# HKUST-KnowComp/DualMessagePassing

Measured on AMD Instinct MI355X. Metric: (pattern,graph) pairs/sec DMPNN fwd+bwd hid=128, higher is better.
Workload: dtype f32

## Files before the change

dualmessagepassing_amd/_abi.py:

```python
import ctypes

c_int = ctypes.c_int
c_i32 = ctypes.c_int32
c_i64 = ctypes.c_int64
c_u64 = ctypes.c_uint64
c_f32 = ctypes.c_float
c_double = ctypes.c_double
c_ptr = ctypes.c_void_p
c_size = ctypes.c_size_t

ABI_VERSION = 92

DMP_COLLATE_MAX_JOBS = 4
DMP_POOL_MAX_JOBS = 4
DMP_REDUCE_MAX_SEGMENTS = 16
DMP_ADAMW_MAX_SKIP = 16
DMP_ADAMW_MAX_SEGMENTS = 1024
DMP_LOOKUP_MAX_JOBS = 8
DMP_CONCAT_MAX_JOBS = 12
DMP_GEMM_MAX_JOBS = 12
DMP_GEMM_MAX_TERMS = 3
DMP_ATB_MAX_JOBS = 8
DMP_MEM_MEAN, DMP_MEM_SUM, DMP_MEM_MAX = 0, 1, 2


class dmp_collate_job(ctypes.Structure):
    _fields_ = [("local_src", c_ptr), ("local_dst", c_ptr), ("num_nodes", c_ptr), ("num_edges", c_ptr), ("B", c_i64), ("N", c_i64),
                ("E", c_i64), ("node_off", c_ptr), ("edge_off", c_ptr), ("src", c_ptr), ("dst", c_ptr), ("edge_graph", c_ptr),
                ("node_graph", c_ptr)]


class dmp_pool_job(ctypes.Structure):
    _fields_ = [("sizes_a", c_ptr), ("sizes_b", c_ptr), ("Ba", c_i64), ("Bb", c_i64), ("flag_a", c_ptr), ("flag_b", c_ptr),
                ("rows_a", c_i64), ("R", c_i64), ("chunk", c_int), ("off", c_ptr), ("gptr", c_ptr), ("vptr", c_ptr), ("vent", c_ptr),
                ("gent", c_ptr), ("seg", c_ptr), ("flag8", c_ptr), ("rowmap", c_ptr), ("sizes", c_ptr)]


class dmp_smallk_job(ctypes.Structure):
    _fields_ = [("X", c_ptr), ("ldx", c_i64), ("D", c_ptr), ("ldd", c_i64), ("gate", c_ptr), ("rowmask", c_ptr), ("R", c_i64),
                ("partial", c_ptr)]


class dmp_l0_pack_job(ctypes.Structure):
    _fields_ = [("enc_p", c_ptr), ("ldp", c_i64), ("rows_p", c_i64), ("enc_g", c_ptr), ("ldg", c_i64), ("gate", c_ptr), ("rows_g", c_i64),
# ... 244 lines not shown
    "dmp_mfma_partial_rows_h": (c_i64, [c_i64, c_int]),
    "dmp_gemm_k64": (c_int, [c_ptr, c_i64, c_ptr, c_i64, c_int, c_ptr, c_i64, c_i64, c_ptr]),
    "dmp_atb_typed": (c_int, [c_ptr, c_i64, c_ptr, c_i64, c_ptr, c_ptr, c_ptr, c_i64, c_i64, c_int, c_ptr, c_ptr, c_ptr]),
    "dmp_out_fwd_fused_rows": (c_int, [c_ptr, c_i64, c_ptr, c_i64, c_ptr, c_ptr, c_ptr, c_int, c_ptr, c_i64, c_i64, c_int, c_int, c_ptr,
                                       c_i64, c_ptr]),
    "dmp_bwd_h1_fused_rows": (c_int, [c_ptr, c_i64, c_ptr, c_i64, c_ptr, c_i64, c_ptr, c_ptr, c_ptr, c_int, c_i64, c_int, c_f32, c_ptr,
                                      c_i64, c_ptr, c_ptr, c_ptr]),
    "dmp_kept_rows_scratch_words": (c_i64, [c_i64]),
    "dmp_kept_rows": (c_int, [c_ptr, c_i64, c_int, c_ptr, c_ptr, c_ptr, c_ptr]),
    "dmp_l0_edge_fwd_rows": (c_int, [c_ptr, c_i64, c_int, c_ptr, c_i64, c_ptr, c_i64, c_ptr, c_ptr, c_ptr, c_ptr, c_ptr, c_ptr, c_i64, c_int,
                                     c_f32, c_ptr, c_i64, c_ptr]),
    "dmp_l0_bwd_w_rows": (c_int, [c_ptr, c_i64, c_int, c_ptr, c_ptr, c_i64, c_ptr, c_i64, c_ptr, c_ptr, c_i64, c_int, c_ptr, c_ptr]),
    "dmp_typed_partial_rows": (c_i64, [c_i64, c_int]),
    "dmp_out_fwd_typed": (c_int, [_p(dmp_typed_job), c_int, c_ptr, c_ptr, c_ptr, c_i64, c_i64, c_int, c_ptr]),
    "dmp_bwd_h1_typed": (c_int, [c_ptr, c_i64, c_ptr, c_i64, c_ptr, c_i64, c_ptr, c_ptr, c_ptr, c_i64, c_i64, c_int, c_f32, c_ptr, c_i64,
                                 c_ptr, c_ptr, c_ptr]),
    "dmp_kept_rows_jobs": (c_int, [_p(dmp_kept_job), c_int, c_ptr, c_ptr, c_ptr, c_ptr, c_i64, c_ptr, c_ptr, c_ptr, c_ptr]),
    "dmp_row_mask_bits_jobs": (c_int, [_p(dmp_rowmask_job), c_int, c_ptr]),
    "dmp_atb2_blocks": (c_i64, [c_i64, c_int]),
    "dmp_atb2_jobs": (c_int, [_p(dmp_atb2_job), c_int, c_ptr, c_ptr, c_ptr, c_i64, c_i64, c_int, c_ptr]),
    "dmp_bwd_z_w": (c_int, [c_ptr, c_i64, c_ptr, c_i64, c_ptr, c_i64, c_ptr, c_i64, c_i64, c_ptr, c_i64, c_ptr, c_ptr, c_f32, c_f32,
                            c_ptr, c_ptr, c_ptr, c_i64, c_i64, c_int, c_ptr, c_i64, c_ptr, c_i64, c_ptr, c_ptr]),
    "dmp_out_fwd_typed_codes": (c_int, [_p(dmp_typed_job), c_ptr, c_i64, c_int, c_ptr, c_i64, c_i64, c_i64, c_ptr, c_ptr, c_ptr, c_i64, c_i64, c_int, c_ptr]),
    "dmp_bwd_h1_w_blocks": (c_i64, [c_i64]),
    "dmp_bwd_h1_w": (c_int, [c_ptr, c_i64, c_ptr, c_i64, c_ptr, c_i64, c_ptr, c_ptr, c_i64, c_i64, c_int, c_f32, c_ptr, c_i64,
                             c_ptr, c_ptr, c_ptr, c_ptr]),
    "dmp_node_chain_blocks": (c_i64, [c_i64]),
    "dmp_node_chain_panel_words": (c_i64, []),
    "dmp_node_chain_pack": (c_int, [_p(dmp_chain_panel), c_int, c_ptr, c_ptr]),
    "dmp_node_chain_fwd": (c_int, [c_ptr, c_i64, c_ptr, c_i64, c_ptr, c_ptr, c_ptr, c_int, c_f32, c_ptr, c_ptr, c_i64, c_i64, c_int,
                                   c_ptr, c_i64, c_ptr, c_i64, c_ptr, c_i64, c_ptr]),
    "dmp_node_chain_bwd": (c_int, [c_ptr, c_i64, c_ptr, c_i64, c_ptr, c_i64, c_ptr, c_int, c_f32, c_ptr, c_ptr, c_i64, c_i64, c_int,
                                   c_ptr, c_i64, c_ptr, c_i64, c_ptr, c_i64, c_ptr, c_ptr, c_ptr]),
    "dmp_row_mask_bits": (c_int, [c_ptr, c_i64, c_ptr, c_ptr]),
    "dmp_row_mask_rows": (c_int, [c_ptr, c_i64, c_int, c_i64, c_ptr, c_ptr]),
    "dmp_bwd_z_fused": (c_int, [c_ptr, c_i64, c_ptr, c_i64, c_ptr, c_i64, c_i64, c_ptr, c_i64, c_ptr, c_ptr, c_ptr,
                                c_f32, c_f32, c_i64, c_int, c_ptr, c_i64, c_ptr]),
    "dmp_gemm_k128": (c_int, [c_ptr, c_i64, c_ptr, c_i64, c_int, c_ptr, c_i64, c_i64, c_int, c_ptr]),
    "dmp_edge_combine": (c_int, [c_ptr, c_i64, c_ptr, c_i64, c_ptr, c_ptr, c_ptr, c_ptr, c_ptr, c_i64,
                                 c_int, c_int, c_f32, c_ptr, c_i64, c_ptr]),
    "dmp_relu_bwd_g_colsum": (c_int, [c_ptr, c_i64, c_ptr, c_i64, c_ptr, c_ptr, c_i64, c_int, c_f32, c_ptr, c_i64,
                                      c_ptr, c_ptr]),
    "dmp_edge_combine_bwd_g": (c_int, [c_ptr, c_i64, c_ptr, c_ptr, c_i64, c_int, c_ptr, c_i64, c_ptr]),
    "dmp_compgcn_agg": (c_int, [c_ptr, c_i64, c_ptr, c_i64, c_ptr, c_ptr, c_ptr, c_ptr, c_i64, c_int, c_int,
                                c_ptr, c_i64, c_ptr]),
    "dmp_compgcn_agg_bwd": (c_int, [c_ptr, c_i64, c_ptr, c_i64, c_ptr, c_i64, c_ptr, c_ptr, c_ptr, c_ptr,
                                    c_i64, c_int, c_int, c_ptr, c_i64, c_ptr, c_i64, c_ptr]),
    "dmp_attn_supported_dh": (c_int, [c_int]),
    "dmp_attn_fwd": (c_int, [c_ptr, c_ptr, c_ptr, c_ptr, c_ptr, c_i64, c_i64, c_i64, c_int, c_int, c_f32, c_ptr, c_ptr, c_ptr, c_ptr]),
    "dmp_attn_bwd": (c_int, [c_ptr, c_ptr, c_ptr, c_ptr, c_ptr, c_ptr, c_ptr, c_ptr, c_i64, c_i64, c_i64, c_int, c_int, c_f32, c_ptr,
                             c_ptr, c_ptr, c_ptr, c_ptr]),
    "dmp_mem_init_fwd": (c_int, [c_ptr, c_i64, c_ptr, c_i64, c_ptr, c_i64, c_i64, c_int, c_int, c_int, c_int, c_int, c_ptr, c_ptr,
                                 c_ptr, c_ptr, c_ptr, c_ptr, c_ptr]),
    "dmp_mem_init_bwd": (c_int, [c_ptr, c_ptr, c_ptr, c_ptr, c_ptr, c_i64, c_i64, c_int, c_int, c_int, c_int, c_ptr, c_ptr, c_ptr]),
    "dmp_cnn_fwd": (c_int, [c_ptr, c_i64, c_i64, c_int, c_ptr, c_ptr, c_int, c_int, c_int, c_int, c_int, c_f32, c_ptr, c_int, c_ptr,
                            c_ptr, c_ptr, c_ptr, c_ptr]),
    "dmp_cnn_route_bwd": (c_int, [c_ptr, c_ptr, c_ptr, c_i64, c_i64, c_i64, c_int, c_int, c_int, c_f32, c_ptr, c_ptr]),
    "dmp_cnn_wgrad_chunks": (c_i64, [c_i64]),
    "dmp_cnn_wgrad": (c_int, [c_ptr, c_ptr, c_i64, c_i64, c_i64, c_int, c_int, c_int, c_ptr, c_ptr]),
    "dmp_rnn_fwd": (c_int, [c_ptr, c_ptr, c_ptr, c_ptr, c_ptr, c_i64, c_i64, c_int, c_int, c_int, c_ptr, c_ptr, c_ptr, c_ptr]),
    "dmp_rnn_bwd": (c_int, [c_ptr, c_ptr, c_ptr, c_ptr, c_ptr, c_i64, c_i64, c_int, c_int, c_int, c_ptr, c_ptr]),
    "dmp_relconv_supported": (c_int, [c_int, c_int]),
    "dmp_relconv_fwd": (c_int, [c_ptr, c_ptr, c_ptr, c_ptr, c_ptr, c_ptr, c_ptr, c_i64, c_int, c_int, c_int, c_int, c_int, c_ptr,
                                c_ptr]),
    "dmp_relconv_bwd": (c_int, [c_ptr, c_ptr, c_ptr, c_ptr, c_ptr, c_ptr, c_ptr, c_i64, c_int, c_int, c_int, c_int, c_int, c_ptr,
                                c_ptr]),
# ... 6 lines not shown
```

dualmessagepassing_amd/_build.py:

```python
import fcntl
import hashlib
import os
import shutil
import subprocess
import tempfile

_HERE = os.path.dirname(os.path.abspath(__file__))
CSRC = os.path.join(_HERE, "csrc")
LIB_PATH = os.path.join(CSRC, "libdmp_hip.so")
HASH_PATH = LIB_PATH + ".srchash"
SOURCES = ["dmp_agg.hip", "dmp_segacc.hip", "dmp_compact.hip", "dmp_graph.hip", "dmp_fused.hip", "dmp_mfma.hip", "dmp_typed.hip", "dmp_h1w.hip", "dmp_nodechain.hip", "dmp_atb.hip", "dmp_fold.hip", "dmp_heads.hip", "dmp_layer0.hip", "dmp_bn.hip", "dmp_attn.hip", "dmp_mem.hip", "dmp_cnn.hip", "dmp_rnn.hip", "dmp_relconv.hip", "dmp_relcorr.hip",
           "dmp_subiso.cpp"]
HEADERS = ["dmp_common.h", "dmp_mfma_common.h", os.path.join("..", "..", "include", "dmp_hip.h")]
ARCH = "gfx950"
FLAGS = ["-O3", "-std=c++17", "-fPIC", "-ffp-contract=off", "-Wall", "-Wno-unused-function"]


def find_hipcc():
    for cand in (os.environ.get("HIPCC"), shutil.which("hipcc"), "/opt/rocm/bin/hipcc"):
        if cand and os.path.exists(cand):
            return cand
    return None


def source_hash():
    h = hashlib.sha256()
    h.update((ARCH + " ".join(FLAGS)).encode())
    for f in SOURCES + HEADERS:
        with open(os.path.join(CSRC, f), "rb") as fh:
            h.update(f.encode())
            h.update(fh.read())
    return h.hexdigest()


def _stale():
    if not os.path.exists(LIB_PATH) or not os.path.exists(HASH_PATH):
        return True
    with open(HASH_PATH) as f:
        return f.read().strip() != source_hash()


def build_lib(force=False, verbose=False):
    if not force and not _stale():
        return LIB_PATH
# ... 43 lines not shown
```

dualmessagepassing_amd/fused.py:

```python
import threading

import torch
from torch.autograd.function import once_differentiable

from . import _abi, _lib, ops
from ._lib import check, ptr, stream_ptr


def _partials(rows, H, dev):
    lib = _lib.load()
    return torch.empty((int(lib.dmp_colsum_partial_rows(rows, H)), H), dtype=torch.float32, device=dev)


MAX_REDUCE_SEGMENTS = _abi.DMP_REDUCE_MAX_SEGMENTS


class _Deferred(threading.local):

    def __init__(self):
        self.stack = []


_deferred = _Deferred()

# ... 617 lines not shown
USE_OUT_CODES = True


def out_codes_ok(h1, enc, K, Wc):
    lib = _lib.load()
    lim = (1 << 32) - 65536
    return bool(USE_OUT_CODES and h1.size(1) == 128 and not lib.dmp_dev_get_exact_fp32() and 1 <= K <= 16 and Wc.size(0) == K and Wc.size(1) == 128
                and enc.dtype == torch.float32 and enc.stride(1) == 1 and enc.stride(0) % 4 == 0 and enc.data_ptr() % 16 == 0
                and enc.size(0) == h1.size(0) and h1.size(0) * 128 * 4 < lim and Wc.stride(1) == 1)


def out_fwd_typed_codes(h1, W2t, b2, enc, K, Wc, tiles, prev=None, out=None, w_in_out=True, row0=0):
    lib = _lib.load()
    slot_edge, tile_scale, num_tiles, bound = tiles
    R, H = h1.shape
    if out is None:
        out = dead_rows_buffer((R, H), h1.device)
    Wc = Wc.detach()
    _lib.require_gpu(h1, W2t, out, prev, b2, enc, Wc)
    j = _abi.dmp_typed_job()
    j.Hin, j.ldh, j.W2, j.ldw, j.w_in_out = h1.data_ptr(), h1.stride(0), W2t.data_ptr(), W2t.stride(0), int(bool(w_in_out))
    j.bias = ptr(b2)
    j.R, j.ldr = ptr(prev), (prev.stride(0) if prev is not None else H)
    j.R2, j.ldr2 = None, H
    j.act, j.slope = 0, 0.0
    j.out, j.ldo = out.data_ptr(), out.stride(0)
    with _lib.timed("out_fwd_typed_codes[H=%d,R=%d]", (H, R), 4 * H * R * 2 + 4 * enc.size(1) * R):
        check(lib.dmp_out_fwd_typed_codes(_ctypes.byref(j), ptr(enc), enc.stride(0), int(K), ptr(Wc), Wc.stride(0), int(row0),
                                          0 if prev is None else min(R, prev.size(0)), ptr(slot_edge), ptr(tile_scale),
                                          ptr(num_tiles), bound, R, H, stream_ptr()), "dmp_out_fwd_typed_codes")
    return out


def out_fwd_typed(h1, W2t, b2, prev, tiles, out=None, w_in_out=True, slope=None, prev2=None):
    R, H = h1.shape
    if out is None:
        out = dead_rows_buffer((R, H), h1.device)
    typed_jobs([dict(a=h1, W=W2t, bias=b2, prev=prev, prev2=prev2, out=out, w_in_out=w_in_out, slope=slope)], tiles)
    return out


def bwd_h1_typed(d_o, W2, h1, tiles, slope=0.0, out=None):
    lib = _lib.load()
    E, H = d_o.shape
    slot_edge, tile_scale, num_tiles, bound = tiles
    d_g = out if out is not None else dead_rows_buffer((E, H), d_o.device)
    G = int(lib.dmp_typed_partial_rows(bound, H))
    part = torch.empty((G, H), dtype=torch.float32, device=d_o.device)
    part_rows = torch.empty_like(part)
    W2 = W2.contiguous()
    with _lib.timed("bwd_h1_typed[H=%d,E=%d]", (H, E), 12 * H * E + 4 * E):
        check(lib.dmp_bwd_h1_typed(ptr(d_o), d_o.stride(0), ptr(W2), W2.size(1), ptr(h1), h1.stride(0), ptr(slot_edge), ptr(tile_scale),
                                   ptr(num_tiles), bound, E, H, slope, ptr(d_g), d_g.stride(0), ptr(part), ptr(part_rows), stream_ptr()),
              "dmp_bwd_h1_typed")
    return d_g, reduce_partials(part), reduce_partials(part_rows)


USE_NODE_CHAIN = True


def node_chain_ok(H, *tensors):
    if not USE_NODE_CHAIN or H != 128 or _lib.load().dmp_dev_get_exact_fp32():
        return False
    lim = (1 << 32) - 65536
    for a in tensors:
        if a is None:
            continue
        if (a.dtype != torch.float32 or a.dim() != 2 or a.stride(1) != 1 or a.stride(0) % 4 or a.stride(0) * 4 > 16383
                or a.data_ptr() % 16 or a.size(0) * a.stride(0) * 4 >= lim):
            return False
    return True

# ... 853 lines not shown
                out_fwd_typed(S[:, H:], Bn[H:], None, XP[:, :H], T, out=H1n, slope=slope, prev2=T1)
        elif l0 is not None and node_pass:
            pass
        elif l0 is not None and l0.venc is not None:
            VK = l0.VK
            XP = torch.empty((N, 3 * H), dtype=torch.float32, device=z.device)
            for t, (n0, n1) in l0.vtables(N):
                smallk_embed(l0.venc[n0:n1, :VK], MV[t * VK:(t + 1) * VK], None, XP[n0:n1], H)
        else:
            XP = x @ Wx
        if (l0 is not None and node_pass) or chained:
            PXr, ldpx = PX, 2 * H
        else:
            PXr, ldpx = XP[:, H:], 3 * H
            if l0 is not None or nd is None:
                H1n = add_bias_relu_(SB, XP[:, :H], bn, slope)
        if chained:
            pass
        elif nd is not None:
            xn = dead_rows_buffer((N, H), z.device) if (inner & 1) else torch.zeros((N, H), dtype=torch.float32, device=z.device)
            if nW2t is not None:
                out_fwd_typed(H1n, nW2t, nb2, x if residual else None, nd.tiles, out=xn)
            else:
                out_fwd_typed(H1n, nW2, nb2, x if residual else None, nd.tiles, out=xn, w_in_out=False)
        elif onepanel_ok(H):
            xn = out_fwd_mfma(H1n, nW2, nb2, v_gate, x if residual else None, nW2t)
        else:
            xn = gate_residual(x if residual else None, torch.addmm(nb2, H1n, nW2.t()), v_gate)
        sums_only = epool is not None and not edge_rows
        zn = None
        side.wait("erows" if l0 is not None else "tiles")
        dead_gate = e_gate if (SKIP_DEAD_ROWS and USE_ROW_MASKS and e_gate is not None and typed_ok(index, H)
                               and gate_row_mask(e_gate) is not None) else None
        if l0 is not None:
            H1e = dead_rows_buffer((z.size(0), H), z.device) if dead_gate is not None else torch.empty((z.size(0), H), dtype=torch.float32, device=z.device)
            for t, rows, _ in tables:
                if rows[1] > rows[0]:
                    l0_edge_fwd(enc0, K0, M0[t * K0:(t + 1) * K0], PXr, ldpx, be, coef, index, slope, rows, H1e,
                                mask=gate_row_mask(dead_gate) if dead_gate is not None else None)
        elif typed_ok(index, H):
            H1e = edge_fwd_typed(z, Wes, PXr, ldpx, be, coef, index, slope, dead_gate=dead_gate, sel=None if nd is None else nd.sel)
        elif mfma_ok(index, H):
            H1e = edge_fwd_mfma(z, Wes, PXr, ldpx, be, coef, index, slope)
        else:
            G = z @ Wes
            H1e = edge_combine_raw(G, 2 * H, PXr, ldpx, be, coef, index, H, relu=True, slope=slope)
            del G
            if not sums_only:
                Oe = torch.addmm(eb2, H1e, eW2.t())
                zn = gate_residual(z if residual else None, Oe, e_gate)
        if zn is None and not sums_only:
            dead = (3 if (inner & 1) else 1) if (dead_gate is not None and zero_rows_gate(e_gate)) else 0
            side.wait("tiles")
            lt = live_tiles(index, coef, e_gate) if (dead == 3 and eW2t is not None) else None
            if lt is not None:
                tl_ = ascending_tiles(e_gate) or lt
                if l0 is not None and residual and getattr(l0, "z_from_codes", False) and out_codes_ok(H1e, l0.enc, l0.K, W0[-l0.K:]):
                    zn = out_fwd_typed_codes(H1e, eW2t, eb2, l0.enc, l0.K, W0[-l0.K:], tl_, prev=l0.z_head, row0=l0.z_head.size(0))
                else:
                    zn = out_fwd_typed(H1e, eW2t, eb2, l0_rows(l0, W0, z) if residual else None, tl_)
            elif (l0 is not None and residual and e_gate is None and getattr(l0, "z_from_codes", False) and eW2t is not None
                  and out_codes_ok(H1e, l0.enc, l0.K, W0[-l0.K:]) and identity_tiles(H1e.size(0), H1e.device) is not None):
                zn = out_fwd_typed_codes(H1e, eW2t, eb2, l0.enc, l0.K, W0[-l0.K:], identity_tiles(H1e.size(0), H1e.device), prev=l0.z_head,
                                         row0=l0.z_head.size(0))
            else:
                zn = out_fwd_mfma(H1e, eW2, eb2, e_gate, l0_rows(l0, W0, z) if residual else None, eW2t, dead_rows=dead)
        ctx.index, ctx.coef, ctx.residual, ctx.H = index, coef, residual, H
        ctx.v_gate, ctx.e_gate, ctx.WesT, ctx.slope = v_gate, e_gate, WesT, slope
        ctx.vpool, ctx.epool = vpool, epool
        ctx.inner = int(inner)
        ctx.nd = nd
        ctx.chain_panels = chain_panels
# ... 330 lines not shown
```

include/dmp_hip.h:

```cpp
#ifndef DMP_HIP_H
#define DMP_HIP_H

#include <stddef.h>
#include <stdint.h>

#ifdef __cplusplus
extern "C" {
#endif

#define DMP_OK 0
#define DMP_ERR_BAD_ARG (-1)
#define DMP_ERR_UNSUPPORTED (-2)
#define DMP_ERR_HIP (-3)

#define DMP_ABI_VERSION 92
int dmp_abi_version(void);
const char *dmp_last_hip_error(void);


size_t dmp_csr_workspace_words(int64_t num_nodes, int64_t num_edges);

int dmp_csr_build(const int64_t *key, const uint8_t *flag, int64_t num_edges,
                  int64_t num_nodes, int32_t *rowptr, int32_t *ent,
                  int32_t *key32, int64_t *degree, int32_t *status,
                  int32_t *ws, void *stream);

size_t dmp_csr_pair_workspace_words(int64_t num_nodes);
int dmp_csr_build_pair(const int64_t *dst, const int64_t *src, const uint8_t *flag, int64_t num_edges, int64_t num_nodes,
                       int32_t *in_ptr, int32_t *in_ent, int32_t *dst32, int64_t *in_deg,
                       int32_t *out_ptr, int32_t *out_ent, int32_t *src32, int64_t *out_deg,
                       int32_t *status, int32_t *ws, void *stream);

int dmp_csr_build_graphs_max_nodes(void);
int dmp_csr_build_graphs(const int64_t *dst, const int64_t *src, const uint8_t *flag, const int64_t *node_off,
                         const int64_t *edge_off, int64_t B, int64_t E, int64_t N, int32_t *in_ptr, int32_t *in_ent,
                         int32_t *dst32, int64_t *in_deg, int32_t *out_ptr, int32_t *out_ent, int32_t *src32,
                         int64_t *out_deg, int32_t *status, void *stream);

int dmp_incidence_build(const int32_t *in_ptr, const int32_t *in_ent,
                        const int32_t *out_ptr, const int32_t *out_ent,
                        int64_t num_nodes, int64_t num_edges, int32_t *inc_ptr,
                        int32_t *inc_ent, void *stream);

int dmp_degree_coef(const int64_t *out_deg, int64_t num_nodes, float *coef,
                    void *stream);

int dmp_collate(const int64_t *local_src, const int64_t *local_dst,
                const int64_t *num_nodes, const int64_t *num_edges,
// ... 447 lines not shown

typedef struct {
  const float *Z; int64_t ldz;
  const float *D; int64_t ldd;
  float *partial_T, *partial_B; int64_t partial_stride; int ldp;
} dmp_atb2_job;
int64_t dmp_atb2_blocks(int64_t tiles_bound, int num_jobs);
int dmp_atb2_jobs(const dmp_atb2_job *jobs, int num_jobs, const int32_t *slot_row, const float *tile_scale, const int32_t *num_tiles,
                  int64_t tiles_bound, int64_t rows, int H, void *stream);

int dmp_bwd_z_w(const float *dPre, int64_t ldp, const float *Z, int64_t ldz, const float *W, int64_t ldw, const float *D, int64_t ldd,
                int64_t num_nodes, const float *base, int64_t ldb, const int32_t *dst, const uint8_t *flag, float s0, float s1,
                const int32_t *slot_edge, const float *tile_scale, const int32_t *num_tiles, int64_t tiles_bound, int64_t E, int H,
                const int32_t *base_map, int64_t base_rows, float *dZ, int64_t ldo, float *partial_w, void *stream);
int64_t dmp_bwd_h1_w_blocks(int64_t tiles_bound);
int dmp_bwd_h1_w(const float *dO, int64_t ldo, const float *W2, int64_t ldw, const float *H1, int64_t ldh,
                 const int32_t *slot_edge, const int32_t *num_tiles, int64_t tiles_bound, int64_t E, int H, float slope,
                 float *dG, int64_t ldg, float *partial, float *partial_rows, float *partial_w, void *stream);

typedef struct {
  const float *W; int64_t ld; int transposed;
} dmp_chain_panel;
int64_t dmp_node_chain_blocks(int64_t tiles_bound);
int64_t dmp_node_chain_panel_words(void);
int dmp_node_chain_pack(const dmp_chain_panel *panels, int num_panels, uint32_t *out, void *stream);
int dmp_node_chain_fwd(const float *x, int64_t ldx, const float *S, int64_t lds, const uint32_t *panels, const float *bn, const float *b2,
                       int residual, float slope, const int32_t *slot, const int32_t *num_tiles, int64_t tiles_bound, int64_t rows, int H,
                       float *H1n, int64_t ldh, float *P, int64_t ldp, float *xn, int64_t ldxn, void *stream);
int dmp_node_chain_bwd(const float *dxn, int64_t ldd, const float *H1n, int64_t ldh, const float *dP, int64_t ldp, const uint32_t *panels,
                       int residual, float slope, const int32_t *slot, const int32_t *num_tiles, int64_t tiles_bound, int64_t rows, int H,
                       float *dPn, int64_t ldn, float *dS, int64_t lds, float *dx, int64_t ldx, float *partial, float *partial_rows,
                       void *stream);

int dmp_bwd_z_fused(const float *dPre, int64_t ldp, const float *W, int64_t ldw,
                    const float *D, int64_t ldd, int64_t num_nodes, const float *base, int64_t ldb,
                    const float *coefE, const int32_t *dst, const uint8_t *flag, float s0,
                    float s1, int64_t num_edges, int H, float *dZ, int64_t ldz, void *stream);

int dmp_edge_fwd_typed(const float *Z, int64_t ldz, const float *W, int64_t ldw, const float *P,
                       int64_t ldp, int64_t num_nodes, const float *bias, const int32_t *selA,
                       const int32_t *selB, const int32_t *slot_edge, const float *tile_scale,
                       const int32_t *num_tiles, int64_t tiles_bound, int64_t num_edges, int H,
                       float slope, float *H1, int64_t ldh, void *stream);
int dmp_mask_slots(const int32_t *slot, int64_t n, const float *gate, int64_t E, int32_t *out, void *stream);
int dmp_bwd_z_typed_arow(const float *dPre, int64_t ldp, const float *W, int64_t ldw, const float *D, int64_t ldd,
                         int64_t num_nodes, const float *base, int64_t ldb, const int32_t *dst, const uint8_t *flag,
                         float s0, float s1, const int32_t *slot_edge, const int32_t *slot_arow, const float *tile_scale,
                         const int32_t *num_tiles, int64_t tiles_bound, int64_t E, int H, int w_transposed,
                         const int32_t *base_map, int64_t base_rows, float *dZ, int64_t ldz, void *stream);

int64_t dmp_atb_typed_blocks_h(int64_t tiles_bound, int H);
int dmp_atb_typed(const float *Z, int64_t ldz, const float *dPre, int64_t ldp,
                  const int32_t *slot_edge, const float *tile_scale, const int32_t *num_tiles,
                  int64_t tiles_bound, int64_t num_edges, int H, float *partial_T,
                  float *partial_B, void *stream);

int64_t dmp_atb_rows_blocks_h(int64_t rows, int M, int N, int H);
int dmp_atb_rows_masked(const float *A, int64_t lda, const float *B, int64_t ldb, const float *gate, const uint32_t *rowmask,
                        int64_t rows, int M, int N, int H, float *partial, float *partial_colsum, void *stream);
int dmp_atb_rows_plain(const float *A, int64_t lda, const float *B, int64_t ldb, const uint32_t *rowmask, int64_t rows, int M, int N,
                       int H, float *partial, void *stream);

int dmp_rel_gemm(const float *A, int64_t lda, int64_t rows_a, const float *W, int64_t ldw, int num_rels,
                 int w_transposed, const int32_t *slot_arow, const int32_t *slot_row,
                 const int32_t *tile_type, const int32_t *num_tiles, int64_t tiles_bound,
                 const float *row_scale, int64_t rows_c, int H, float *C, int64_t ldc, void *stream);
// ... 75 lines not shown
```

Measured before the change: 494,000.

## Fuse edge MLP first layer and output layer into one warp-specialized kernel

Adds a new HIP kernel that computes the edge first layer (typed GEMM plus gathered node terms, bias, activation) in four waves and pipes the activated tile through LDS to four other waves that run the second GEMM with bias and residual. The forward path uses it when the gated, residual, odd-inner-layer conditions hold. The aim is to avoid a separate launch and a global round trip of H1 into the second GEMM. In exchange the kernel is complex, runs one 512-thread block per CU with large LDS, and the two wave groups' throughput must stay balanced.

```diff
diff --git a/dualmessagepassing_amd/_abi.py b/dualmessagepassing_amd/_abi.py
--- a/dualmessagepassing_amd/_abi.py
+++ b/dualmessagepassing_amd/_abi.py
@@ -9,7 +9,7 @@
 c_ptr = ctypes.c_void_p
 c_size = ctypes.c_size_t
 
-ABI_VERSION = 92
+ABI_VERSION = 93
 
 DMP_COLLATE_MAX_JOBS = 4
 DMP_POOL_MAX_JOBS = 4
@@ -320,6 +320,8 @@
                                    c_ptr, c_i64, c_ptr, c_i64, c_ptr, c_i64, c_ptr]),
     "dmp_node_chain_bwd": (c_int, [c_ptr, c_i64, c_ptr, c_i64, c_ptr, c_i64, c_ptr, c_int, c_f32, c_ptr, c_ptr, c_i64, c_i64, c_int,
                                    c_ptr, c_i64, c_ptr, c_i64, c_ptr, c_i64, c_ptr, c_ptr, c_ptr]),
+    "dmp_edge_mlp_fwd": (c_int, [c_ptr, c_i64, c_ptr, c_i64, c_ptr, c_i64, c_i64, c_ptr, c_ptr, c_ptr, c_ptr, c_i64, c_int, c_ptr, c_ptr, c_i64,
+                                 c_ptr, c_ptr, c_ptr, c_i64, c_i64, c_int, c_f32, c_ptr, c_i64, c_ptr, c_i64, c_ptr]),
     "dmp_row_mask_bits": (c_int, [c_ptr, c_i64, c_ptr, c_ptr]),
     "dmp_row_mask_rows": (c_int, [c_ptr, c_i64, c_int, c_i64, c_ptr, c_ptr]),
     "dmp_bwd_z_fused": (c_int, [c_ptr, c_i64, c_ptr, c_i64, c_ptr, c_i64, c_i64, c_ptr, c_i64, c_ptr, c_ptr, c_ptr,
diff --git a/dualmessagepassing_amd/_build.py b/dualmessagepassing_amd/_build.py
--- a/dualmessagepassing_amd/_build.py
+++ b/dualmessagepassing_amd/_build.py
@@ -9,7 +9,7 @@
 CSRC = os.path.join(_HERE, "csrc")
 LIB_PATH = os.path.join(CSRC, "libdmp_hip.so")
 HASH_PATH = LIB_PATH + ".srchash"
-SOURCES = ["dmp_agg.hip", "dmp_segacc.hip", "dmp_compact.hip", "dmp_graph.hip", "dmp_fused.hip", "dmp_mfma.hip", "dmp_typed.hip", "dmp_h1w.hip", "dmp_nodechain.hip", "dmp_atb.hip", "dmp_fold.hip", "dmp_heads.hip", "dmp_layer0.hip", "dmp_bn.hip", "dmp_attn.hip", "dmp_mem.hip", "dmp_cnn.hip", "dmp_rnn.hip", "dmp_relconv.hip", "dmp_relcorr.hip",
+SOURCES = ["dmp_agg.hip", "dmp_segacc.hip", "dmp_compact.hip", "dmp_graph.hip", "dmp_fused.hip", "dmp_mfma.hip", "dmp_typed.hip", "dmp_h1w.hip", "dmp_nodechain.hip", "dmp_edgemlp.hip", "dmp_atb.hip", "dmp_fold.hip", "dmp_heads.hip", "dmp_layer0.hip", "dmp_bn.hip", "dmp_attn.hip", "dmp_mem.hip", "dmp_cnn.hip", "dmp_rnn.hip", "dmp_relconv.hip", "dmp_relcorr.hip",
            "dmp_subiso.cpp"]
 HEADERS = ["dmp_common.h", "dmp_mfma_common.h", os.path.join("..", "..", "include", "dmp_hip.h")]
 ARCH = "gfx950"
diff --git a/dualmessagepassing_amd/csrc/dmp_edgemlp.hip b/dualmessagepassing_amd/csrc/dmp_edgemlp.hip
--- /dev/null
+++ b/dualmessagepassing_amd/csrc/dmp_edgemlp.hip
@@ -0,0 +1,366 @@
+#include "dmp_mfma_common.h"
+
+namespace dmp {
+namespace {
+
+struct EdgeMlpArgs {
+  const float *Z; int64_t ldz;
+  const float *W; int64_t ldw;
+  const float *P; int64_t ldp; int64_t num_nodes;
+  const float *bias1;
+  const int32_t *selA, *selB;
+  const float *W2; int64_t ldw2; int w2_transposed;
+  const float *bias2;
+  const float *R; int64_t ldr;
+  float *H1; int64_t ldh;
+  float *out; int64_t ldo;
+  int64_t E;
+  const int32_t *slot_edge;
+  const float *tile_scale;
+  const int32_t *num_tiles;
+  float slope;
+};
+
+constexpr int kHE = 128, kThreadsE = 512;
+constexpr int kStrideD = (kHE + 8) / 2;
+constexpr int kPlaneD = kSub * kStrideD;
+constexpr int kTileD = 3 * kPlaneD;
+constexpr int kRing = 4;
+constexpr int kImgOffH = 2 * kTileD * 4;
+constexpr int kScrOff = 4 * kTileD * 4;
+constexpr int kRowsOff = kScrOff + 8 * 32 * kScrStride * 4;
+constexpr int kEdgeMlpLdsBytes = kRowsOff + 3 * kRing * kSub * 4;
+constexpr int kHalfE = kHE / 2, kGroupsE = kHalfE / 8;
+
+__global__ __launch_bounds__(kThreadsE, 1) void edge_mlp_k(const EdgeMlpArgs p) {
+  extern __shared__ __attribute__((aligned(16))) unsigned char lds[];
+  uint32_t *const zimg = reinterpret_cast<uint32_t *>(lds);
+  uint32_t *const himg = reinterpret_cast<uint32_t *>(lds + kImgOffH);
+  uint32_t *const rowA = reinterpret_cast<uint32_t *>(lds + kRowsOff);
+  uint32_t *const rowB = rowA + kRing * kSub, *const rowC = rowB + kRing * kSub;
+  const int wave = __builtin_amdgcn_readfirstlane((int)(threadIdx.x >> 6));
+  const bool second = wave >= 4;
+  const int lane = threadIdx.x & 63, li = lane & 31, h = lane >> 5, cs = wave & 3;
+  const int gtid = threadIdx.x & 255;
+  const int col = 32 * cs + li;
+  float *const scr = reinterpret_cast<float *>(lds + kScrOff) + wave * (32 * kScrStride);
+  const int lrow = lane >> 3, c4 = 32 * cs + (lane & 7) * 4;
+  const uint32_t col4 = (uint32_t)c4 * 4u;
+  constexpr uint32_t kRowBytes = kHE * 4u;
+  constexpr uint32_t kNone = 0xFFFFFFFFu, kOOB = 0xFFFFF000u;
+
+  const int ntiles = __builtin_amdgcn_readfirstlane(*p.num_tiles);
+  const int chunk = (ntiles + (int)gridDim.x - 1) / (int)gridDim.x;
+  const int lo = (int)blockIdx.x * chunk;
+  const int hi = lo + chunk < ntiles ? lo + chunk : ntiles;
+  const int mine = hi > lo ? hi - lo : 0;
+  if (mine == 0) return;
+
+  Split8 B6[kGroupsE];
+  f32x16 acc;
+  auto x6_tile = [&](const uint32_t *img, auto &&action) {
+#pragma unroll
+    for (int r = 0; r < 16; ++r) acc[r] = 0.f;
+    const uint32_t *ar = img + li * kStrideD + (kHalfE / 2) * h;
+    Frag8 ah, am, al;
+    ah.v = *reinterpret_cast<const bf16x8 *>(ar);
+    am.v = *reinterpret_cast<const bf16x8 *>(ar + kPlaneD);
+    al.v = *reinterpret_cast<const bf16x8 *>(ar + 2 * kPlaneD);
+#pragma unroll
+    for (int g = 0; g < kGroupsE; ++g) {
+      Frag8 nh = ah, nm = am, nl = al;
+      if (g + 1 < kGroupsE) {
+        nh.v = *reinterpret_cast<const bf16x8 *>(ar + 4 * (g + 1));
+        nm.v = *reinterpret_cast<const bf16x8 *>(ar + kPlaneD + 4 * (g + 1));
+        nl.v = *reinterpret_cast<const bf16x8 *>(ar + 2 * kPlaneD + 4 * (g + 1));
+      }
+      const Split8 &bb = B6[g];
+      __builtin_amdgcn_sched_barrier(0);
+      acc = __builtin_amdgcn_mfma_f32_32x32x16_bf16(al.v, bb.hi.v, acc, 0, 0, 0);
+      acc = __builtin_amdgcn_mfma_f32_32x32x16_bf16(ah.v, bb.lo.v, acc, 0, 0, 0);
+      acc = __builtin_amdgcn_mfma_f32_32x32x16_bf16(am.v, bb.mid.v, acc, 0, 0, 0);
+      __builtin_amdgcn_sched_barrier(0);
+      action(2 * g);
+      __builtin_amdgcn_sched_barrier(0);
+      acc = __builtin_amdgcn_mfma_f32_32x32x16_bf16(am.v, bb.hi.v, acc, 0, 0, 0);
+      acc = __builtin_amdgcn_mfma_f32_32x32x16_bf16(ah.v, bb.mid.v, acc, 0, 0, 0);
+      acc = __builtin_amdgcn_mfma_f32_32x32x16_bf16(ah.v, bb.hi.v, acc, 0, 0, 0);
+      __builtin_amdgcn_sched_barrier(0);
+      action(2 * g + 1);
+      ah = nh; am = nm; al = nl;
+    }
+  };
+  auto acc_to_scr = [&]() {
+#pragma unroll
+    for (int r = 0; r < 16; ++r) scr[((r & 3) + 8 * (r >> 2) + 4 * h) * kScrStride + li] = acc[r];
+  };
+
+  if (!second) {
+    float4 bias4 = make_float4(0.f, 0.f, 0.f, 0.f);
+    if (p.bias1) bias4 = *reinterpret_cast<const float4 *>(p.bias1 + c4);
+    const float slope = __builtin_bit_cast(float, __builtin_amdgcn_readfirstlane(__builtin_bit_cast(int, p.slope)));
+    const uint32_t rows4 = (uint32_t)(p.E * 4);
+    const srsrc_t rs_Z = make_srsrc(p.Z, p.ldz, p.E);
+    const srsrc_t rs_H1 = make_srsrc(p.H1, p.ldh, p.E);
+    const srsrc_t rs_T = make_srsrc(p.P, p.ldp, p.num_nodes);
+    const rsrc_t rs_idxA = make_rsrc(p.selA, rows4);
+    const rsrc_t rs_idxB = make_rsrc(p.selB, rows4);
+    const rsrc_t rs_slot = make_rsrc(p.slot_edge, (uint32_t)ntiles * (kSub * 4u));
+    const uint32_t colA = (uint32_t)(gtid & 31) * 16u;
+    const int srow = gtid >> 5;
+
+    const rsrc_t rs_W = make_rsrc(p.W, (uint32_t)(kHE * p.ldw * 4));
+    const uint32_t w_first = (uint32_t)((int64_t)kHalfE * h * p.ldw + col) * 4u;
+    const uint32_t w_step = __builtin_amdgcn_readfirstlane((int)(p.ldw * 4));
+    auto load_panel = [&](float c) {
+      uint32_t off, ws;
+      asm volatile("v_mov_b32 %0, %1" : "=v"(off) : "v"(w_first));
+      asm volatile("s_mov_b32 %0, %1" : "=s"(ws) : "s"(w_step));
+#pragma unroll
+      for (int s0 = 0; s0 < kHalfE; s0 += 32) {
+        float w0[32], w1[32];
+#pragma unroll
+        for (int j = 0; j < 32; ++j) {
+          w0[j] = __uint_as_float(__builtin_amdgcn_raw_buffer_load_b32(rs_W, (int)off, (int)((s0 + j) * ws), 0));
+          w1[j] = __uint_as_float(__builtin_amdgcn_raw_buffer_load_b32(rs_W, (int)off + (int)kRowBytes, (int)((s0 + j) * ws), 0));
+        }
+#pragma unroll
+        for (int q = 0; q < 32; q += 8) {
+          float w[8];
+#pragma unroll
+          for (int j = 0; j < 8; ++j) w[j] = w0[q + j] + c * w1[q + j];
+          split8(make_float4(w[0], w[1], w[2], w[3]), make_float4(w[4], w[5], w[6], w[7]), B6[(s0 + q) / 8]);
+        }
+        __builtin_amdgcn_sched_barrier(0);
+      }
+    };
+
+    int id_rows[kSubLoads];
+    int id_own = -1, own_staged = -1;
+    float4 pre[kSubLoads];
+    uint32_t pre_a = 0, pre_b = 0;
+    auto load_ids = [&](int k) {
+      const bool ok = k < mine;
+      const uint32_t so = (uint32_t)(lo + k) * (kSub * 4u);
+#pragma unroll
+      for (int m = 0; m < kSubLoads; ++m)
+        id_rows[m] = ok ? (int)__builtin_amdgcn_raw_buffer_load_b32(rs_slot, (srow + 8 * m) * 4, (int)so, 0) : -1;
+      if (gtid < kSub) id_own = ok ? (int)__builtin_amdgcn_raw_buffer_load_b32(rs_slot, gtid * 4, (int)so, 0) : -1;
+    };
+    auto load_row = [&](int m) { pre[m] = sbuf_load4(rs_Z, id_rows[m], colA); };
+    auto load_row_scalars = [&]() {
+      if (gtid < kSub) {
+        const uint32_t eo = id_own >= 0 ? (uint32_t)id_own * 4u : kOOB;
+        pre_a = __builtin_amdgcn_raw_buffer_load_b32(rs_idxA, (int)eo, 0, 0);
+        pre_b = __builtin_amdgcn_raw_buffer_load_b32(rs_idxB, (int)eo, 0, 0);
+        own_staged = id_own;
+      }
+    };
+    auto stage_row = [&](int buf, int m) {
+      uint2 ph, pm, pl;
+      split_pair(pre[m].x, pre[m].y, ph.x, pm.x, pl.x);
+      split_pair(pre[m].z, pre[m].w, ph.y, pm.y, pl.y);
+      uint32_t *q = zimg + buf * kTileD + (srow + 8 * m) * kStrideD + (gtid & 31) * 2;
+      *reinterpret_cast<uint2 *>(q) = ph;
+      *reinterpret_cast<uint2 *>(q + kPlaneD) = pm;
+      *reinterpret_cast<uint2 *>(q + 2 * kPlaneD) = pl;
+    };
+    auto stage_scalars = [&](int par) {
+      if (gtid < kSub) {
+        const bool ok = own_staged >= 0;
+        rowA[par * kSub + gtid] = ok ? pre_a : kNone;
+        rowB[par * kSub + gtid] = ok ? pre_b : kNone;
+        rowC[par * kSub + gtid] = ok ? (uint32_t)own_staged : kNone;
+      }
+    };
+    float4 g0[4], g1[4];
+    auto fetch_operand = [&](int par, int k) {
+      const int rr = 8 * k + lrow;
+      g0[k] = sbuf_load4(rs_T, (int)rowA[par * kSub + rr], col4);
+      g1[k] = sbuf_load4(rs_T, (int)rowB[par * kSub + rr], col4 + kRowBytes);
+    };
+    auto tile_step = [&](int k, int par) {
+      const int buf = k & 1, nxt = (par + 1) & (kRing - 1);
+      x6_tile(zimg + buf * kTileD, [&](int i) {
+        if (i < 4) {}
+        else if (i < 8) stage_row(buf ^ 1, i - 4);
+        else if (i == 8) stage_scalars(nxt);
+        else if (i < 13) load_row(i - 9);
+        else if (i == 13) load_row_scalars();
+        else if (i == 14) load_ids(k + 3);
+      });
+    };
+    auto epilogue = [&](int k, int par) {
+      uint32_t *const img = himg + (k & 1) * kTileD;
+      const int nxt = (par + 1) & (kRing - 1);
+      acc_to_scr();
+#pragma unroll
+      for (int q = 0; q < 4; ++q) {
+        const int rr = 8 * q + lrow;
+        float4 v = *reinterpret_cast<const float4 *>(&scr[rr * kScrStride + (lane & 7) * 4]);
+        v.x = act_fwd((v.x + (g0[q].x - g1[q].x)) + bias4.x, slope);
+        v.y = act_fwd((v.y + (g0[q].y - g1[q].y)) + bias4.y, slope);
+        v.z = act_fwd((v.z + (g0[q].z - g1[q].z)) + bias4.z, slope);
+        v.w = act_fwd((v.w + (g0[q].w - g1[q].w)) + bias4.w, slope);
+        const uint32_t rc = rowC[par * kSub + rr];
+        sbuf_store4(v, rs_H1, (int)rc, col4);
+        const bool pad = rc == kNone;
+        uint2 ph, pm, pl;
+        split_pair(pad ? 0.f : v.x, pad ? 0.f : v.y, ph.x, pm.x, pl.x);
+        split_pair(pad ? 0.f : v.z, pad ? 0.f : v.w, ph.y, pm.y, pl.y);
+        uint32_t *w = img + rr * kStrideD + (c4 >> 1);
+        *reinterpret_cast<uint2 *>(w) = ph;
+        *reinterpret_cast<uint2 *>(w + kPlaneD) = pm;
+        *reinterpret_cast<uint2 *>(w + 2 * kPlaneD) = pl;
+        fetch_operand(nxt, q);
+      }
+    };
+
+    load_ids(0);
+#pragma unroll
+    for (int m = 0; m < kSubLoads; ++m) load_row(m);
+    load_row_scalars();
+    load_ids(1);
+    float c_have = p.tile_scale[lo];
+    load_panel(c_have);
+#pragma unroll
+    for (int m = 0; m < kSubLoads; ++m) stage_row(0, m);
+    stage_scalars(0);
+#pragma unroll
+    for (int m = 0; m < kSubLoads; ++m) load_row(m);
+    load_row_scalars();
+    load_ids(2);
+    lds_barrier();
+#pragma unroll
+    for (int c = 0; c < 4; ++c) fetch_operand(0, c);
+    int k = 0, par = 0;
+    float sv = 0.f;
+    unsigned long long starts = 0;
+    while (k < mine) {
+      if ((k & 63) == 0) {
+        const float last = __shfl(sv, 63);
+        sv = k + lane < mine ? p.tile_scale[lo + k + lane] : 0.f;
+        float up = __shfl_up(sv, 1);
+        if (lane == 0) up = k > 0 ? last : sv;
+        starts = __ballot(k + lane < mine && __float_as_uint(sv) != __float_as_uint(up));
+      }
+      const float c = __shfl(sv, k & 63);
+      if (__float_as_uint(c) != __float_as_uint(c_have)) {
+        load_panel(c);
+        c_have = c;
+      }
+      do {
+        tile_step(k, par);
+        lds_barrier();
+        epilogue(k, par);
+        ++k;
+        par = (par + 1) & (kRing - 1);
+      } while (k < mine && (k & 63) != 0 && ((starts >> (k & 63)) & 1ull) == 0);
+    }
+    lds_barrier();
+  } else {
+    __builtin_amdgcn_s_setprio(1);
+    float4 bias4 = make_float4(0.f, 0.f, 0.f, 0.f);
+    if (p.bias2) bias4 = *reinterpret_cast<const float4 *>(p.bias2 + c4);
+    const srsrc_t rs_R = make_srsrc(p.R, p.R ? p.ldr : (int64_t)kHE, p.E);
+    const srsrc_t rs_O = make_srsrc(p.out, p.ldo, p.E);
+    {
+      const rsrc_t rs_W = make_rsrc(p.W2, (uint32_t)(kHE * p.ldw2 * 4));
+      const uint32_t w_first = (uint32_t)(p.w2_transposed ? (int64_t)col * p.ldw2 + kHalfE * h : (int64_t)kHalfE * h * p.ldw2 + col) * 4u;
+      const uint32_t w_step = __builtin_amdgcn_readfirstlane((int)(p.w2_transposed ? 4 : p.ldw2 * 4));
+      uint32_t off;
+      asm volatile("v_mov_b32 %0, %1" : "=v"(off) : "v"(w_first));
+#pragma unroll
+      for (int s0 = 0; s0 < kHalfE; s0 += 32) {
+        float w0[32];
+#pragma unroll
+        for (int j = 0; j < 32; ++j) w0[j] = __uint_as_float(__builtin_amdgcn_raw_buffer_load_b32(rs_W, (int)off, (int)((s0 + j) * w_step), 0));
+#pragma unroll
+        for (int q = 0; q < 32; q += 8)
+          split8(make_float4(w0[q], w0[q + 1], w0[q + 2], w0[q + 3]), make_float4(w0[q + 4], w0[q + 5], w0[q + 6], w0[q + 7]), B6[(s0 + q) / 8]);
+        __builtin_amdgcn_sched_barrier(0);
+      }
+    }
+    float4 g1[4];
+    auto fetch_residual = [&](int par, int q) {
+      g1[q] = sbuf_load4(rs_R, (int)rowC[par * kSub + 8 * q + lrow], col4);
+    };
+    lds_barrier();
+#pragma unroll
+    for (int q = 0; q < 4; ++q) fetch_residual(0, q);
+    lds_barrier();
+    int par = 0;
+    for (int k = 0; k < mine; ++k) {
+      lds_barrier();
+      x6_tile(himg + (k & 1) * kTileD, [&](int) {});
+      acc_to_scr();
+      const int nxt = (par + 1) & (kRing - 1);
+#pragma unroll
+      for (int q = 0; q < 4; ++q) {
+        const int rr = 8 * q + lrow;
+        float4 v = *reinterpret_cast<const float4 *>(&scr[rr * kScrStride + (lane & 7) * 4]);
+        v.x = (v.x + bias4.x) + g1[q].x; v.y = (v.y + bias4.y) + g1[q].y;
+        v.z = (v.z + bias4.z) + g1[q].z; v.w = (v.w + bias4.w) + g1[q].w;
+        sbuf_store4(v, rs_O, (int)rowC[par * kSub + rr], col4);
+        fetch_residual(nxt, q);
+      }
+      par = nxt;
+    }
+  }
+}
+
+inline unsigned edge_mlp_blocks(int64_t tiles_bound) {
+  const int64_t cap = 256;
+  return (unsigned)(tiles_bound < cap ? (tiles_bound > 0 ? tiles_bound : 1) : cap);
+}
+
+constexpr int kMaxDevicesE = 64;
+inline bool edge_mlp_lds_ready() {
+  static bool done[kMaxDevicesE] = {};
+  int dev = 0;
+  if (hipGetDevice(&dev) != hipSuccess || dev < 0 || dev >= kMaxDevicesE) dev = 0;
+  if (done[dev]) return true;
+  const hipError_t e = hipFuncSetAttribute(reinterpret_cast<const void *>(&edge_mlp_k), hipFuncAttributeMaxDynamicSharedMemorySize, kEdgeMlpLdsBytes);
+  if (e != hipSuccess) { set_last_hip_error(e); return false; }
+  done[dev] = true;
+  return true;
+}
+
+}
+}
+
+using namespace dmp;
+
+extern "C" {
+
+int dmp_edge_mlp_fwd(const float *Z, int64_t ldz, const float *W, int64_t ldw, const float *P, int64_t ldp, int64_t num_nodes,
+                     const float *bias1, const int32_t *selA, const int32_t *selB, const float *W2, int64_t ldw2, int w2_in_out,
+                     const float *bias2, const float *R, int64_t ldr, const int32_t *slot_edge, const float *tile_scale,
+                     const int32_t *num_tiles, int64_t tiles_bound, int64_t E, int H, float slope, float *H1, int64_t ldh,
+                     float *out, int64_t ldo, void *stream) {
+  if (H != 128 || g_exact_fp32) return DMP_ERR_UNSUPPORTED;
+  if (E < 0 || num_nodes < 0 || tiles_bound < 0) return DMP_ERR_BAD_ARG;
+  if (!slope_ok(slope)) return DMP_ERR_UNSUPPORTED;
+  if (E == 0 || tiles_bound == 0) return DMP_OK;
+  if (!Z || !W || !P || !selA || !selB || !W2 || !slot_edge || !tile_scale || !num_tiles || !H1 || !out || ldz < H || ldw < 2 * H ||
+      ldp < 2 * H || ldw2 < H || ldh < H || ldo < H || (R && ldr < H))
+    return DMP_ERR_BAD_ARG;
+  if (ldz % 4 || ldh % 4 || ldp % 4 || ldo % 4 || (R && ldr % 4) || !aligned16(Z) || !aligned16(H1) || !aligned16(P) || !aligned16(out) ||
+      (R && !aligned16(R)) || (bias1 && !aligned16(bias1)) || (bias2 && !aligned16(bias2)))
+    return DMP_ERR_UNSUPPORTED;
+  const int64_t lim32 = ((int64_t)1 << 32) - 8192;
+  if (!stride_ok(ldz) || !stride_ok(ldh) || !stride_ok(ldp) || !stride_ok(ldo) || (R && !stride_ok(ldr)) || E >= ((int64_t)1 << 30) ||
+      num_nodes >= ((int64_t)1 << 31) || tiles_bound * kSub * 4 >= lim32 || (int64_t)H * ldw * 4 >= lim32 || (int64_t)H * ldw2 * 4 >= lim32 ||
+      !fits4g(E, ldz) || !fits4g(E, ldh) || !fits4g(E, ldo) || (R && !fits4g(E, ldr)) || !fits4g(num_nodes, ldp))
+    return DMP_ERR_UNSUPPORTED;
+  if (!edge_mlp_lds_ready()) return DMP_ERR_HIP;
+  EdgeMlpArgs a{};
+  a.Z = Z; a.ldz = ldz; a.W = W; a.ldw = ldw; a.P = P; a.ldp = ldp; a.num_nodes = num_nodes; a.bias1 = bias1; a.selA = selA; a.selB = selB;
+  a.W2 = W2; a.ldw2 = ldw2; a.w2_transposed = w2_in_out ? 0 : 1; a.bias2 = bias2; a.R = R; a.ldr = R ? ldr : H;
+  a.H1 = H1; a.ldh = ldh; a.out = out; a.ldo = ldo; a.E = E; a.slot_edge = slot_edge; a.tile_scale = tile_scale; a.num_tiles = num_tiles;
+  a.slope = slope;
+  edge_mlp_k<<<edge_mlp_blocks(tiles_bound), kThreadsE, kEdgeMlpLdsBytes, (hipStream_t)stream>>>(a);
+  return check_launch();
+}
+
+}
diff --git a/dualmessagepassing_amd/fused.py b/dualmessagepassing_amd/fused.py
--- a/dualmessagepassing_amd/fused.py
+++ b/dualmessagepassing_amd/fused.py
@@ -673,12 +673,53 @@
     return out
 
 
-def out_fwd_typed(h1, W2t, b2, prev, tiles, out=None, w_in_out=True, slope=None, prev2=None):
+def out_fwd_typed(h1, W2t, b2, prev, tiles, out=None, w_in_out=True, slope=None, prev2=None, first=None):
     R, H = h1.shape
     if out is None:
         out = dead_rows_buffer((R, H), h1.device)
+    if first is not None:
+        if prev2 is not None or slope is not None:
+            raise _lib.DmpError("out_fwd_typed(first=...): neither a second addend nor an activation on the result")
+        edge_mlp_fwd(first["z"], first["Wes"], first["P"], first["ldp"], first["bias"], first["coef"], first["index"], first["slope"],
+                     W2t, b2, prev, tiles, sel=first.get("sel"), w_in_out=w_in_out, h1=h1, out=out)
+        return out
     typed_jobs([dict(a=h1, W=W2t, bias=b2, prev=prev, prev2=prev2, out=out, w_in_out=w_in_out, slope=slope)], tiles)
     return out
+
+
+USE_EDGE_MLP_FWD = True
+
+
+def edge_mlp_fwd_ok(H, *tensors):
+    if not USE_EDGE_MLP_FWD or H != 128 or _lib.load().dmp_dev_get_exact_fp32():
+        return False
+    lim = (1 << 32) - 65536
+    for a in tensors:
+        if a is None:
+            continue
+        if (a.dtype != torch.float32 or a.dim() != 2 or a.stride(1) != 1 or a.stride(0) % 4 or a.stride(0) * 4 > 16383
+                or a.data_ptr() % 16 or a.size(0) * a.stride(0) * 4 >= lim):
+            return False
+    return True
+
+
+def edge_mlp_fwd(z, Wes, P, ldp, bias, coef, index, slope, W2t, b2, prev, tiles, sel=None, w_in_out=True, h1=None, out=None):
+    lib = _lib.load()
+    E, H = z.shape
+    slot_edge, tile_scale, num_tiles, bound = tiles
+    if h1 is None:
+        h1 = dead_rows_buffer((E, H), z.device)
+    if out is None:
+        out = dead_rows_buffer((E, H), z.device)
+    Wes = Wes.contiguous()
+    sel_a, sel_b = (sel[0], sel[1]) if sel is not None else index.edge_select(coef)[:2]
+    _lib.require_gpu(z, Wes, P, bias, W2t, b2, prev, h1, out)
+    with _lib.timed("edge_fwd_typed[H=%d,E=%d]", (H, E), 4 * H * (2 * E + 2 * index.num_nodes) + 12 * E):
+        check(lib.dmp_edge_mlp_fwd(ptr(z), z.stride(0), ptr(Wes), Wes.size(1), ptr(P), ldp, index.num_nodes, ptr(bias), ptr(sel_a), ptr(sel_b),
+                                   ptr(W2t), W2t.stride(0), int(bool(w_in_out)), ptr(b2), ptr(prev), prev.stride(0) if prev is not None else H,
+                                   ptr(slot_edge), ptr(tile_scale), ptr(num_tiles), bound, E, H, float(slope), ptr(h1), h1.stride(0),
+                                   ptr(out), out.stride(0), stream_ptr()), "dmp_edge_mlp_fwd")
+    return h1, out
 
 
 def bwd_h1_typed(d_o, W2, h1, tiles, slope=0.0, out=None):
@@ -1598,12 +1639,21 @@
         side.wait("erows" if l0 is not None else "tiles")
         dead_gate = e_gate if (SKIP_DEAD_ROWS and USE_ROW_MASKS and e_gate is not None and typed_ok(index, H)
                                and gate_row_mask(e_gate) is not None) else None
+        mlp_tiles = None
+        if (l0 is None and dead_gate is not None and not sums_only and residual and eW2t is not None and (inner & 1)
+                and zero_rows_gate(e_gate) and edge_mlp_fwd_ok(H, z, PXr, eW2t)):
+            mlp_tiles = live_tiles(index, coef, e_gate)
         if l0 is not None:
             H1e = dead_rows_buffer((z.size(0), H), z.device) if dead_gate is not None else torch.empty((z.size(0), H), dtype=torch.float32, device=z.device)
             for t, rows, _ in tables:
                 if rows[1] > rows[0]:
                     l0_edge_fwd(enc0, K0, M0[t * K0:(t + 1) * K0], PXr, ldpx, be, coef, index, slope, rows, H1e,
                                 mask=gate_row_mask(dead_gate) if dead_gate is not None else None)
+        elif mlp_tiles is not None:
+            H1e = dead_rows_buffer((z.size(0), H), z.device)
+            zn = out_fwd_typed(H1e, eW2t, eb2, z, mlp_tiles,
+                               first=dict(z=z, Wes=Wes, P=PXr, ldp=ldpx, bias=be, coef=coef, index=index, slope=slope,
+                                          sel=None if nd is None else nd.sel))
         elif typed_ok(index, H):
             H1e = edge_fwd_typed(z, Wes, PXr, ldpx, be, coef, index, slope, dead_gate=dead_gate, sel=None if nd is None else nd.sel)
         elif mfma_ok(index, H):
diff --git a/include/dmp_hip.h b/include/dmp_hip.h
--- a/include/dmp_hip.h
+++ b/include/dmp_hip.h
@@ -13,7 +13,7 @@
 #define DMP_ERR_UNSUPPORTED (-2)
 #define DMP_ERR_HIP (-3)
 
-#define DMP_ABI_VERSION 92
+#define DMP_ABI_VERSION 93
 int dmp_abi_version(void);
 const char *dmp_last_hip_error(void);
 
@@ -527,6 +527,12 @@
                        float *dPn, int64_t ldn, float *dS, int64_t lds, float *dx, int64_t ldx, float *partial, float *partial_rows,
                        void *stream);
 
+int dmp_edge_mlp_fwd(const float *Z, int64_t ldz, const float *W, int64_t ldw, const float *P, int64_t ldp, int64_t num_nodes,
+                     const float *bias1, const int32_t *selA, const int32_t *selB, const float *W2, int64_t ldw2, int w2_in_out,
+                     const float *bias2, const float *R, int64_t ldr, const int32_t *slot_edge, const float *tile_scale,
+                     const int32_t *num_tiles, int64_t tiles_bound, int64_t num_edges, int H, float slope, float *H1, int64_t ldh,
+                     float *out, int64_t ldo, void *stream);
+
 int dmp_bwd_z_fused(const float *dPre, int64_t ldp, const float *W, int64_t ldw,
                     const float *D, int64_t ldd, int64_t num_nodes, const float *base, int64_t ldb,
                     const float *coefE, const int32_t *dst, const uint8_t *flag, float s0,
```

New measurement: 499,100 (median of 6 runs). 1.01x the previous value.
